# akashsengupta1997/STRAPS-3DHumanShapePose

Measured on AMD Instinct MI355X. Metric: bodies/sec, higher is better.
Workload: dtype fp32 (encoder convolutions as exact bf16x3 operand splits (six bf16 products per term); in-step SMPL blend contraction and skinning as 3-product fp16 splits (fp16x3_lbs: 22-bit operands); fp32 accumulate throughout)

## Files before the change

straps-3dhumanshapepose_amd/csrc/smpl_bwd.hip:

```cpp
#include "common.h"
#include "rodrigues.h"

namespace {

constexpr int KP = STRAPS_SMPL_KP, KG = KP / 8, NT = STRAPS_SMPL_TILES, NV = STRAPS_SMPL_V, NROUNDS = NT / 4;
constexpr int BT = 32, AS = 292, SS = 193;
constexpr int NJS = STRAPS_SMPL_NPICK + STRAPS_SMPL_NEXTRA;

__global__ __launch_bounds__(256, 1) STRAPS_NO_PACKED_FP32 void smpl_verts_bwd_kernel(straps_smpl_model_t m, const float* __restrict__ F,
                                                                const float* __restrict__ Amat, const float* __restrict__ dverts,
                                                                const float* __restrict__ djoints, float* __restrict__ dFp,
                                                                float* __restrict__ dAp, long long B, int rounds_per_chunk) {
    extern __shared__ __attribute__((aligned(16))) float smem[];
    float* As_ = smem;
    float* stage = As_ + BT * AS;

    const int tid = threadIdx.x, lane = tid & 63, wave = tid >> 6;
    const int h = lane >> 5, bl = lane & 31;
    const int chunk = blockIdx.x;
    const long long b0 = (long long)blockIdx.y * BT;
    const int nb = (int)((B - b0) < BT ? (B - b0) : BT);

    for (int i = tid; i < BT * 72; i += 256) {
        const int b = i / 72, q = i % 72;
        f32x4 v = {0.f, 0.f, 0.f, 0.f};
        if (b < nb) v = *reinterpret_cast<const f32x4*>(Amat + (b0 + b) * 288 + q * 4);
        *reinterpret_cast<f32x4*>(As_ + b * AS + q * 4) = v;
    }
    __syncthreads();

    const int round0 = chunk * rounds_per_chunk;
    const int round1 = min(round0 + rounds_per_chunk, NROUNDS);
    const f32x4* __restrict__ blend = reinterpret_cast<const f32x4*>(m.blend_frag);
    const f32x4* __restrict__ blend_t = reinterpret_cast<const f32x4*>(m.blend_frag_t);
    float* mystage = stage + wave * BT * SS;
    const int KW = m.skin_k;
    const bool vbody = bl < nb;

    float dacc[3][12];
#pragma unroll
    for (int i = 0; i < 3; ++i)
#pragma unroll
        for (int e = 0; e < 12; ++e) dacc[i][e] = 0.f;
    f32x16 accF[7];
#pragma unroll
    for (int f = 0; f < 7; ++f)
#pragma unroll
        for (int q = 0; q < 16; ++q) accF[f][q] = 0.f;

    for (int rd = round0; rd < round1; ++rd) {
        const int tile = rd * 4 + wave;
        f32x16 ax, ay, az;
#pragma unroll
        for (int r = 0; r < 16; ++r) { ax[r] = 0.f; ay[r] = 0.f; az[r] = 0.f; }
        {
            const f32x4* px = blend + ((long long)(tile * 3 + 0) * KG) * 64 + lane;
            const f32x4* py = px + KG * 64;
            const f32x4* pz = py + KG * 64;
            const float* frow = F + (b0 + (vbody ? bl : 0)) * KP + 4 * h;
            f32x4 cx0 = px[0], cy0 = py[0], cz0 = pz[0];
            f32x4 fn = *reinterpret_cast<const f32x4*>(frow);
#pragma unroll 2
            for (int g = 0; g < KG; ++g) {
                f32x4 nx0 = cx0, ny0 = cy0, nz0 = cz0;
                const f32x4 f0 = vbody ? fn : f32x4{0.f, 0.f, 0.f, 0.f};
                if (g + 1 < KG) {
                    nx0 = px[(g + 1) * 64]; ny0 = py[(g + 1) * 64]; nz0 = pz[(g + 1) * 64];
                    fn = *reinterpret_cast<const f32x4*>(frow + 8 * (g + 1));
                }
#pragma unroll
                for (int e = 0; e < 4; ++e) {
                    ax = mfma32(cx0[e], f0[e], ax);
                    ay = mfma32(cy0[e], f0[e], ay);
                    az = mfma32(cz0[e], f0[e], az);
                }
                cx0 = nx0; cy0 = ny0; cz0 = nz0;
            }
        }
        {
            const int ncol = min(96, (NV - tile * 32) * 3);
            for (int i = lane; i < BT * 96; i += 64) {
                const int b = i / 96, c = i - b * 96;
                float v = 0.f;
                if (dverts && b < nb && c < ncol) v = dverts[(b0 + b) * (long long)(NV * 3) + tile * 96 + c];
                mystage[b * SS + (c / 3) * 6 + (c % 3)] = v;
            }
        }
        __syncthreads();
        if (djoints && h == 0 && vbody) {
            const float* dj = djoints + (b0 + bl) * (STRAPS_SMPL_NJOINTS_OUT * 3) + 72;
            const int e0 = m.jrt_ptr[tile], e1 = m.jrt_ptr[tile + 1];
            for (int e = e0; e < e1; ++e) {
                const int code = m.jrt_code[e];
                const float w = m.jrt_w[e];
                float* sv = mystage + bl * SS + (code >> 8) * 6;
                const float* g = dj + (code & 255) * 3;
                sv[0] = fmaf(w, g[0], sv[0]); sv[1] = fmaf(w, g[1], sv[1]); sv[2] = fmaf(w, g[2], sv[2]);
            }
        }
        __syncthreads();
        {
            const float* Ab = As_ + bl * AS;
#pragma unroll
            for (int r = 0; r < 16; ++r) {
                const int vrow = (r & 3) + 8 * (r >> 2) + 4 * h;
                const int v = tile * 32 + vrow;
                float* sv = mystage + bl * SS + vrow * 6;
                const float gx = sv[0], gy = sv[1], gz = sv[2];
                sv[3] = ax[r]; sv[4] = ay[r]; sv[5] = az[r];
                float t00 = 0.f, t01 = 0.f, t02 = 0.f, t10 = 0.f, t11 = 0.f, t12 = 0.f, t20 = 0.f, t21 = 0.f, t22 = 0.f;
                for (int k = 0; k < KW; ++k) {
                    const float w = m.skin_w[v * KW + k];
                    const int jo = m.skin_j[v * KW + k] * 12;
                    const f32x4 a0 = *reinterpret_cast<const f32x4*>(Ab + jo);
                    const f32x4 a1 = *reinterpret_cast<const f32x4*>(Ab + jo + 4);
                    const f32x4 a2 = *reinterpret_cast<const f32x4*>(Ab + jo + 8);
                    t00 += w * a0[0]; t01 += w * a0[1]; t02 += w * a0[2];
                    t10 += w * a1[0]; t11 += w * a1[1]; t12 += w * a1[2];
                    t20 += w * a2[0]; t21 += w * a2[1]; t22 += w * a2[2];
                }
                ax[r] = t00 * gx + t10 * gy + t20 * gz;
                ay[r] = t01 * gx + t11 * gy + t21 * gz;
                az[r] = t02 * gx + t12 * gy + t22 * gz;
            }
        }
        __syncthreads();
#pragma unroll
        for (int i = 0; i < 3; ++i) {
            const int j = wave + 4 * (2 * i + h);
            const int e0 = m.dj_ptr[rd * 24 + j], e1 = m.dj_ptr[rd * 24 + j + 1];
            for (int e = e0; e < e1; ++e) {
                const int code = m.dj_code[e];
                const float w = m.dj_w[e];
                const float* sv = stage + ((code >> 5) * BT + bl) * SS + (code & 31) * 6;
                const float wx = w * sv[0], wy = w * sv[1], wz = w * sv[2];
                const float x = sv[3], y = sv[4], z = sv[5];
                dacc[i][0] = fmaf(wx, x, dacc[i][0]); dacc[i][1] = fmaf(wx, y, dacc[i][1]); dacc[i][2] = fmaf(wx, z, dacc[i][2]); dacc[i][3] += wx;
                dacc[i][4] = fmaf(wy, x, dacc[i][4]); dacc[i][5] = fmaf(wy, y, dacc[i][5]); dacc[i][6] = fmaf(wy, z, dacc[i][6]); dacc[i][7] += wy;
                dacc[i][8] = fmaf(wz, x, dacc[i][8]); dacc[i][9] = fmaf(wz, y, dacc[i][9]); dacc[i][10] = fmaf(wz, z, dacc[i][10]); dacc[i][11] += wz;
            }
        }
        {
            const f32x4* pt = blend_t + ((long long)tile * 3 * 7 * 4) * 64 + lane;
#pragma unroll
            for (int c = 0; c < 3; ++c) {
#pragma unroll
                for (int f = 0; f < 7; ++f) {
#pragma unroll
                    for (int rq = 0; rq < 4; ++rq) {
                        const f32x4 a = pt[((c * 7 + f) * 4 + rq) * 64];
#pragma unroll
                        for (int e = 0; e < 4; ++e) {
                            const float g = c == 0 ? ax[rq * 4 + e] : (c == 1 ? ay[rq * 4 + e] : az[rq * 4 + e]);
                            accF[f] = mfma32(a[e], g, accF[f]);
                        }
                    }
                }
            }
        }
        __syncthreads();
    }
    {
        __syncthreads();
        float* red = smem;
        if (wave >= 2) {
#pragma unroll
            for (int f = 0; f < 7; ++f)
#pragma unroll
                for (int q = 0; q < 16; ++q) red[(wave - 2) * 7168 + (f * 16 + q) * 64 + lane] = accF[f][q];
        }
        __syncthreads();
        if (wave < 2) {
#pragma unroll
            for (int f = 0; f < 7; ++f)
#pragma unroll
                for (int q = 0; q < 16; ++q) accF[f][q] += red[wave * 7168 + (f * 16 + q) * 64 + lane];
        }
        __syncthreads();
        if (wave == 1) {
#pragma unroll
            for (int f = 0; f < 7; ++f)
#pragma unroll
                for (int q = 0; q < 16; ++q) red[(f * 16 + q) * 64 + lane] = accF[f][q];
        }
        __syncthreads();
        if (wave == 0) {
#pragma unroll
            for (int f = 0; f < 7; ++f)
#pragma unroll
                for (int q = 0; q < 16; ++q) accF[f][q] += red[(f * 16 + q) * 64 + lane];
        }
    }
    if (vbody && wave == 0) {
        float* o = dFp + ((long long)chunk * B + b0 + bl) * KP;
#pragma unroll
        for (int f = 0; f < 7; ++f)
#pragma unroll
            for (int q = 0; q < 16; ++q) o[f * 32 + mfma_row(q, lane)] = accF[f][q];
    }
    if (vbody) {
        float* o = dAp + ((long long)chunk * B + b0 + bl) * 288;
#pragma unroll
        for (int i = 0; i < 3; ++i) {
            const int j = wave + 4 * (2 * i + h);
#pragma unroll
            for (int e = 0; e < 12; ++e) o[j * 12 + e] = dacc[i][e];
        }
    }
}

__device__ __forceinline__ float lane_get(float value, int src) { return __shfl(value, src, 64); }
template <bool AA>
__global__ __launch_bounds__(256) STRAPS_NO_PACKED_FP32 void smpl_pose_bwd_kernel(straps_smpl_model_t m, const float* __restrict__ betas,
                                                            const float* __restrict__ rotmats, const float* __restrict__ dFp,
                                                            const float* __restrict__ dAp, const float* __restrict__ djoints,
                                                            float* __restrict__ dbetas, float* __restrict__ drot, long long B,
                                                            int chunks, const float* __restrict__ aa, float* __restrict__ daa) {
    const int lane = threadIdx.x & 63;
    const int j = lane & 31;
    const int base = lane & 32;
    const long long body = ((long long)blockIdx.x * 256 + threadIdx.x) >> 5;
    const bool vb = body < B;
    const bool vj = j < 24;
    const long long bb = vb ? body : 0;
    const int jj = vj ? j : 0;

    float beta[10];
#pragma unroll
    for (int l = 0; l < 10; ++l) beta[l] = betas[bb * 10 + l];
    float R[9];
#pragma unroll
    for (int e = 0; e < 9; ++e) R[e] = rotmats[(bb * 24 + jj) * 9 + e];
    float J[3];
#pragma unroll
    for (int c = 0; c < 3; ++c) {
        float s = m.j_template[jj * 3 + c];
#pragma unroll
        for (int l = 0; l < 10; ++l) s = fmaf(m.j_shapedirs[(jj * 3 + c) * 10 + l], beta[l], s);
        J[c] = s;
    }
    const int par = m.parents[jj];
    const int dep = vj ? m.depth[jj] : -1;
    const int src = base + (par < 0 ? 0 : par);
    float rel[3];
#pragma unroll
    for (int c = 0; c < 3; ++c) {
        const float jp = lane_get(J[c], src);
        rel[c] = (jj > 0) ? J[c] - jp : J[c];
    }
    float G[12], PR[9];
#pragma unroll
    for (int r = 0; r < 3; ++r) {
        G[r * 4 + 0] = R[r * 3 + 0]; G[r * 4 + 1] = R[r * 3 + 1]; G[r * 4 + 2] = R[r * 3 + 2]; G[r * 4 + 3] = rel[r];
    }
#pragma unroll
    for (int e = 0; e < 9; ++e) PR[e] = (e == 0 || e == 4 || e == 8) ? 1.f : 0.f;
    for (int d = 1; d <= m.max_depth; ++d) {
        float P[12];
#pragma unroll
        for (int e = 0; e < 12; ++e) P[e] = lane_get(G[e], src);
        if (dep == d) {
#pragma unroll
            for (int r = 0; r < 3; ++r) {
                const float p0 = P[r * 4 + 0], p1 = P[r * 4 + 1], p2 = P[r * 4 + 2];
                PR[r * 3 + 0] = p0; PR[r * 3 + 1] = p1; PR[r * 3 + 2] = p2;
                G[r * 4 + 0] = p0 * R[0] + p1 * R[3] + p2 * R[6];
                G[r * 4 + 1] = p0 * R[1] + p1 * R[4] + p2 * R[7];
                G[r * 4 + 2] = p0 * R[2] + p1 * R[5] + p2 * R[8];
                G[r * 4 + 3] = p0 * rel[0] + p1 * rel[1] + p2 * rel[2] + P[r * 4 + 3];
            }
        }
    }
    float gA[12];
#pragma unroll
    for (int e = 0; e < 12; ++e) gA[e] = 0.f;
    if (vb && vj)
        for (int c = 0; c < chunks; ++c) {
            const float* p = dAp + (((long long)c * B + body) * 24 + j) * 12;
#pragma unroll
            for (int e = 0; e < 12; ++e) gA[e] += p[e];
        }
    float gGR[9], gGt[3], gJ[3];
#pragma unroll
    for (int r = 0; r < 3; ++r) {
        const float gat = gA[r * 4 + 3];
        gGR[r * 3 + 0] = gA[r * 4 + 0] - gat * J[0];
        gGR[r * 3 + 1] = gA[r * 4 + 1] - gat * J[1];
        gGR[r * 3 + 2] = gA[r * 4 + 2] - gat * J[2];
        gGt[r] = gat + ((vb && vj && djoints) ? djoints[(body * STRAPS_SMPL_NJOINTS_OUT + j) * 3 + r] : 0.f);
    }
#pragma unroll
    for (int c = 0; c < 3; ++c) gJ[c] = -(G[0 * 4 + c] * gA[3] + G[1 * 4 + c] * gA[7] + G[2 * 4 + c] * gA[11]);

    int child[3];
#pragma unroll
    for (int c = 0; c < 3; ++c) child[c] = m.children[jj * 3 + c];
    float gR[9];
#pragma unroll
    for (int e = 0; e < 9; ++e) gR[e] = 0.f;
    for (int d = m.max_depth; d >= 1; --d) {
        float M[15];
        const bool mine = (dep == d);
        float grel[3];
#pragma unroll
        for (int c = 0; c < 3; ++c) grel[c] = PR[0 * 3 + c] * gGt[0] + PR[1 * 3 + c] * gGt[1] + PR[2 * 3 + c] * gGt[2];
#pragma unroll
        for (int r = 0; r < 3; ++r)
#pragma unroll
            for (int c = 0; c < 3; ++c)
                M[r * 3 + c] = mine ? (gGR[r * 3 + 0] * R[c * 3 + 0] + gGR[r * 3 + 1] * R[c * 3 + 1] + gGR[r * 3 + 2] * R[c * 3 + 2] + gGt[r] * rel[c]) : 0.f;
#pragma unroll
        for (int c = 0; c < 3; ++c) { M[9 + c] = mine ? gGt[c] : 0.f; M[12 + c] = mine ? -grel[c] : 0.f; }
        if (mine) {
#pragma unroll
            for (int r = 0; r < 3; ++r)
#pragma unroll
                for (int c = 0; c < 3; ++c)
                    gR[r * 3 + c] = PR[0 * 3 + r] * gGR[0 * 3 + c] + PR[1 * 3 + r] * gGR[1 * 3 + c] + PR[2 * 3 + r] * gGR[2 * 3 + c];
#pragma unroll
            for (int c = 0; c < 3; ++c) gJ[c] += grel[c];
        }
#pragma unroll
        for (int cc = 0; cc < 3; ++cc) {
            const int ch = child[cc];
            const int cs = base + (ch < 0 ? 0 : ch);
            float in[15];
#pragma unroll
            for (int e = 0; e < 15; ++e) in[e] = lane_get(M[e], cs);
            if (vj && ch >= 0) {
#pragma unroll
                for (int e = 0; e < 9; ++e) gGR[e] += in[e];
#pragma unroll
                for (int c = 0; c < 3; ++c) { gGt[c] += in[9 + c]; gJ[c] += in[12 + c]; }
            }
        }
    }
    if (j == 0) {
#pragma unroll
        for (int e = 0; e < 9; ++e) gR[e] = gGR[e];
#pragma unroll
        for (int c = 0; c < 3; ++c) gJ[c] += gGt[c];
    }
    float gbeta_direct = 0.f;
    if (vb && vj) {
        for (int c = 0; c < chunks; ++c) {
            const float* p = dFp + ((long long)c * B + body) * KP;
            if (j >= 1) {
#pragma unroll
                for (int e = 0; e < 9; ++e) gR[e] += p[11 + (j - 1) * 9 + e];
            }
            if (j < 10) gbeta_direct += p[1 + j];
        }
        if (!AA || drot) {
#pragma unroll
            for (int e = 0; e < 9; ++e) drot[(body * 24 + j) * 9 + e] = gR[e];
        }
        if constexpr (AA) {
            float ox, oy, oz;
            const float* r = aa + (body * 24 + j) * 3;
            straps_rodrigues_bwd_one(r[0], r[1], r[2], gR, ox, oy, oz);
            float* o = daa + (body * 24 + j) * 3;
            o[0] = ox; o[1] = oy; o[2] = oz;
        }
    }
#pragma unroll
    for (int l = 0; l < 10; ++l) {
        float s = vj ? (m.j_shapedirs[(jj * 3 + 0) * 10 + l] * gJ[0] + m.j_shapedirs[(jj * 3 + 1) * 10 + l] * gJ[1] +
                        m.j_shapedirs[(jj * 3 + 2) * 10 + l] * gJ[2]) : 0.f;
#pragma unroll
        for (int o = 16; o > 0; o >>= 1) s += __shfl_xor(s, o, 64);
        const float direct = lane_get(gbeta_direct, base + l);
        if (vb && j == l) dbetas[body * 10 + l] = s + direct;
    }
}

inline int resolve_rpc(long long batch, int chunks) {
    if (chunks <= 0) chunks = (batch >= 1024) ? 8 : 54;
    if (chunks > NROUNDS) chunks = NROUNDS;
    return (NROUNDS + chunks - 1) / chunks;
}

}

int straps_smpl_launch_pose(const straps_smpl_model_t* model, const float* betas, const float* rotmats, float* F, float* Amat,
                            float* joints, long long batch, hipStream_t st);

extern "C" size_t straps_smpl_bwd_workspace_bytes(long long batch, int chunks) {
    const int rpc = resolve_rpc(batch, chunks);
    const int nch = (NROUNDS + rpc - 1) / rpc;
    return (size_t)batch * (size_t)(KP + 288 + nch * (KP + 288)) * sizeof(float);
}

namespace {
template <bool AA>
int smpl_bwd_launch(const straps_smpl_model_t* model, const float* betas, const float* rotmats, const float* aa, const float* dverts,
                    const float* djoints, float* dbetas, float* drotmats, float* daa, void* workspace, long long batch, int chunks,
                    void* stream) {
    hipStream_t st = (hipStream_t)stream;
    const int rpc = resolve_rpc(batch, chunks);
    const int nch = (NROUNDS + rpc - 1) / rpc;
    float* F = (float*)workspace;
    float* Amat = F + batch * KP;
    float* dFp = Amat + batch * 288;
    float* dAp = dFp + (long long)nch * batch * KP;
    int rc = straps_smpl_launch_pose(model, betas, rotmats, F, Amat, nullptr, batch, st);
    if (rc != STRAPS_OK) return rc;
    const size_t lds = (size_t)(BT * AS + 4 * BT * SS) * sizeof(float);
    STRAPS_RAISE_LDS((smpl_verts_bwd_kernel), lds, "smpl_verts_bwd_kernel");
    const long long btiles = (batch + BT - 1) / BT;
    if (btiles > 65535) { straps_set_error("straps_smpl_bwd: batch %lld exceeds one launch; split it", batch); return STRAPS_EUNSUPPORTED; }
    hipLaunchKernelGGL(smpl_verts_bwd_kernel, dim3(nch, (unsigned)btiles), dim3(256), lds, st, *model, F, Amat, dverts, djoints, dFp, dAp, batch, rpc);
    STRAPS_CHECK_LAUNCH("smpl_verts_bwd_kernel");
    hipLaunchKernelGGL(smpl_pose_bwd_kernel<AA>, dim3((unsigned)((batch * 32 + 255) / 256)), dim3(256), 0, st, *model, betas, rotmats, dFp, dAp,
                       djoints, dbetas, drotmats, batch, nch, aa, daa);
    STRAPS_CHECK_LAUNCH("smpl_pose_bwd_kernel");
    return STRAPS_OK;
}
}

extern "C" int straps_smpl_bwd(const straps_smpl_model_t* model, const float* betas, const float* rotmats, const float* dverts,
                               const float* djoints, float* dbetas, float* drotmats, void* workspace, long long batch, int chunks,
                               void* stream) {
    STRAPS_REQUIRE(model && betas && rotmats && dbetas && drotmats && workspace, "straps_smpl_bwd: null pointer");
    STRAPS_REQUIRE(model->blend_frag_t && model->children && model->jrt_ptr && model->dj_ptr && model->dj_code && model->dj_w,
                   "straps_smpl_bwd: model lacks the backward tables");
    STRAPS_REQUIRE(batch > 0, "straps_smpl_bwd: batch must be positive");
    return smpl_bwd_launch<false>(model, betas, rotmats, nullptr, dverts, djoints, dbetas, drotmats, nullptr, workspace, batch, chunks, stream);
}

extern "C" int straps_smpl_bwd_aa(const straps_smpl_model_t* model, const float* betas, const float* rotmats, const float* full_pose_aa,
                                  const float* dverts, const float* djoints, float* dbetas, float* dfull_pose_aa, float* drotmats,
                                  void* workspace, long long batch, int chunks, void* stream) {
    STRAPS_REQUIRE(model && betas && rotmats && full_pose_aa && dbetas && dfull_pose_aa && workspace, "straps_smpl_bwd_aa: null pointer");
    STRAPS_REQUIRE(model->blend_frag_t && model->children && model->jrt_ptr && model->dj_ptr && model->dj_code && model->dj_w,
                   "straps_smpl_bwd_aa: model lacks the backward tables");
    STRAPS_REQUIRE(batch > 0, "straps_smpl_bwd_aa: batch must be positive");
    return smpl_bwd_launch<true>(model, betas, rotmats, full_pose_aa, dverts, djoints, dbetas, drotmats, dfull_pose_aa, workspace, batch, chunks,
                                 stream);
}
```

Measured before the change: 7889.

## Software-pipeline SMPL backward loads with register rings and prefetched partial reductions

Restructures the vertex backward kernel so the blend and F operands are prefetched into RD-deep register rings with fully unrolled MFMA loops. The dverts tile is loaded into registers early and stored while the MFMAs run, and skinning weights and indices are preloaded. The blend_t MFMA stage also uses a RT-deep ring, the dj edge loop is batched in groups of EB, and __syncthreads is swapped for LDS-only fence barriers. The pose kernel now double-buffers the chunked dAp/dFp partial-sum reads in batches of PU. These changes are meant to hide global memory latency, at the cost of much higher register pressure and possible spills.

New measurement: 7979 (median of 6 runs). 1.01x the previous value.

```diff
diff --git a/straps-3dhumanshapepose_amd/csrc/smpl_bwd.hip b/straps-3dhumanshapepose_amd/csrc/smpl_bwd.hip
--- a/straps-3dhumanshapepose_amd/csrc/smpl_bwd.hip
+++ b/straps-3dhumanshapepose_amd/csrc/smpl_bwd.hip
@@ -6,6 +6,15 @@
 constexpr int KP = STRAPS_SMPL_KP, KG = KP / 8, NT = STRAPS_SMPL_TILES, NV = STRAPS_SMPL_V, NROUNDS = NT / 4;
 constexpr int BT = 32, AS = 292, SS = 193;
 constexpr int NJS = STRAPS_SMPL_NPICK + STRAPS_SMPL_NEXTRA;
+constexpr int RD = 4, RT = 4 * RD, SKP = 4, EB = 8;
+constexpr int PU = 9;
+static_assert(RD >= 1 && RT <= 84, "the rings are filled before their loops");
+
+__device__ __forceinline__ STRAPS_NO_PACKED_FP32 void lds_barrier() {
+    __builtin_amdgcn_fence(__ATOMIC_RELEASE, "workgroup", "local");
+    __builtin_amdgcn_s_barrier();
+    __builtin_amdgcn_fence(__ATOMIC_ACQUIRE, "workgroup", "local");
+}
 
 __global__ __launch_bounds__(256, 1) STRAPS_NO_PACKED_FP32 void smpl_verts_bwd_kernel(straps_smpl_model_t m, const float* __restrict__ F,
                                                                 const float* __restrict__ Amat, const float* __restrict__ dverts,
@@ -50,47 +59,84 @@
 
     for (int rd = round0; rd < round1; ++rd) {
         const int tile = rd * 4 + wave;
+        const f32x4* px = blend + ((long long)(tile * 3 + 0) * KG) * 64 + lane;
+        const f32x4* py = px + KG * 64;
+        const f32x4* pz = py + KG * 64;
+        int fo = (vbody ? bl : 0) * KP + 4 * h;
+        asm volatile("" : "+v"(fo));
+        const float* frow = F + b0 * KP + fo;
+        f32x4 rx[RD], ry[RD], rz[RD], rf[RD];
+#pragma unroll
+        for (int s = 0; s < RD; ++s) {
+            if (s < KG) {
+                rx[s] = px[s * 64]; ry[s] = py[s * 64]; rz[s] = pz[s * 64];
+                rf[s] = *reinterpret_cast<const f32x4*>(frow + 8 * s);
+            }
+        }
+        const int ncol = min(96, (NV - tile * 32) * 3);
+        const float* dvp[3];
+        int dvn[3], dvq[3], dvs[3];
+#pragma unroll
+        for (int u = 0; u < 3; ++u) {
+            const int i0 = lane + 64 * u, bu = i0 >= 96, c = i0 - 96 * bu;
+            dvn[u] = (dverts && c < ncol) ? (nb - bu + 1) / 2 : 0;
+            dvp[u] = dvn[u] > 0 ? dverts + (b0 + bu) * (long long)(NV * 3) + tile * 96 + c : F;
+            dvq[u] = dvn[u] > 0 ? 2 * NV * 3 : 0;
+            dvs[u] = bu * SS + (c / 3) * 6 + (c % 3);
+        }
+        float dvr[48];
+#pragma unroll
+        for (int q = 0; q < 16; ++q) {
+#pragma unroll
+            for (int u = 0; u < 3; ++u) dvr[3 * q + u] = dvp[u][min(q, max(dvn[u] - 1, 0)) * dvq[u]];
+        }
+        const int jr0 = m.jrt_ptr[tile], jr1 = m.jrt_ptr[tile + 1];
+        int de0[3], de1[3];
+#pragma unroll
+        for (int i = 0; i < 3; ++i) {
+            const int j = wave + 4 * (2 * i + h);
+            de0[i] = m.dj_ptr[rd * 24 + j]; de1[i] = m.dj_ptr[rd * 24 + j + 1];
+        }
         f32x16 ax, ay, az;
 #pragma unroll
         for (int r = 0; r < 16; ++r) { ax[r] = 0.f; ay[r] = 0.f; az[r] = 0.f; }
-        {
-            const f32x4* px = blend + ((long long)(tile * 3 + 0) * KG) * 64 + lane;
-            const f32x4* py = px + KG * 64;
-            const f32x4* pz = py + KG * 64;
-            const float* frow = F + (b0 + (vbody ? bl : 0)) * KP + 4 * h;
-            f32x4 cx0 = px[0], cy0 = py[0], cz0 = pz[0];
-            f32x4 fn = *reinterpret_cast<const f32x4*>(frow);
-#pragma unroll 2
-            for (int g = 0; g < KG; ++g) {
-                f32x4 nx0 = cx0, ny0 = cy0, nz0 = cz0;
-                const f32x4 f0 = vbody ? fn : f32x4{0.f, 0.f, 0.f, 0.f};
-                if (g + 1 < KG) {
-                    nx0 = px[(g + 1) * 64]; ny0 = py[(g + 1) * 64]; nz0 = pz[(g + 1) * 64];
-                    fn = *reinterpret_cast<const f32x4*>(frow + 8 * (g + 1));
-                }
-#pragma unroll
-                for (int e = 0; e < 4; ++e) {
-                    ax = mfma32(cx0[e], f0[e], ax);
-                    ay = mfma32(cy0[e], f0[e], ay);
-                    az = mfma32(cz0[e], f0[e], az);
-                }
-                cx0 = nx0; cy0 = ny0; cz0 = nz0;
-            }
-        }
-        {
-            const int ncol = min(96, (NV - tile * 32) * 3);
-            for (int i = lane; i < BT * 96; i += 64) {
-                const int b = i / 96, c = i - b * 96;
-                float v = 0.f;
-                if (dverts && b < nb && c < ncol) v = dverts[(b0 + b) * (long long)(NV * 3) + tile * 96 + c];
-                mystage[b * SS + (c / 3) * 6 + (c % 3)] = v;
-            }
-        }
-        __syncthreads();
+        __builtin_amdgcn_sched_barrier(0);
+#pragma unroll
+        for (int g = 0; g < KG; ++g) {
+            const int s = g % RD;
+            const f32x4 f0 = vbody ? rf[s] : f32x4{0.f, 0.f, 0.f, 0.f};
+#pragma unroll
+            for (int e = 0; e < 4; ++e) {
+                ax = mfma32(rx[s][e], f0[e], ax);
+                ay = mfma32(ry[s][e], f0[e], ay);
+                az = mfma32(rz[s][e], f0[e], az);
+            }
+            if (g + RD < KG) {
+                rx[s] = px[(g + RD) * 64]; ry[s] = py[(g + RD) * 64]; rz[s] = pz[(g + RD) * 64];
+                rf[s] = *reinterpret_cast<const f32x4*>(frow + 8 * (g + RD));
+            }
+            if (g == (RD < KG ? RD : KG) - 1) {
+#pragma unroll
+                for (int t = 0; t < 48; ++t)
+                    mystage[(t / 3) * 2 * SS + dvs[t % 3]] = t / 3 < dvn[t % 3] ? dvr[t] : 0.f;
+            }
+            __builtin_amdgcn_sched_barrier(0);
+        }
+        float skw[16][SKP];
+        int skj[16][SKP];
+#pragma unroll
+        for (int k = 0; k < SKP; ++k) {
+#pragma unroll
+            for (int r = 0; r < 16; ++r) {
+                const int v = tile * 32 + (r & 3) + 8 * (r >> 2) + 4 * h;
+                const int at = k < KW ? v * KW + k : 0;
+                skw[r][k] = m.skin_w[at]; skj[r][k] = m.skin_j[at];
+            }
+        }
+        lds_barrier();
         if (djoints && h == 0 && vbody) {
             const float* dj = djoints + (b0 + bl) * (STRAPS_SMPL_NJOINTS_OUT * 3) + 72;
-            const int e0 = m.jrt_ptr[tile], e1 = m.jrt_ptr[tile + 1];
-            for (int e = e0; e < e1; ++e) {
+            for (int e = jr0; e < jr1; ++e) {
                 const int code = m.jrt_code[e];
                 const float w = m.jrt_w[e];
                 float* sv = mystage + bl * SS + (code >> 8) * 6;
@@ -98,7 +144,7 @@
                 sv[0] = fmaf(w, g[0], sv[0]); sv[1] = fmaf(w, g[1], sv[1]); sv[2] = fmaf(w, g[2], sv[2]);
             }
         }
-        __syncthreads();
+        lds_barrier();
         {
             const float* Ab = As_ + bl * AS;
 #pragma unroll
@@ -109,7 +155,20 @@
                 const float gx = sv[0], gy = sv[1], gz = sv[2];
                 sv[3] = ax[r]; sv[4] = ay[r]; sv[5] = az[r];
                 float t00 = 0.f, t01 = 0.f, t02 = 0.f, t10 = 0.f, t11 = 0.f, t12 = 0.f, t20 = 0.f, t21 = 0.f, t22 = 0.f;
-                for (int k = 0; k < KW; ++k) {
+#pragma unroll
+                for (int k = 0; k < SKP; ++k) {
+                    if (k < KW) {
+                        const float w = skw[r][k];
+                        const int jo = skj[r][k] * 12;
+                        const f32x4 a0 = *reinterpret_cast<const f32x4*>(Ab + jo);
+                        const f32x4 a1 = *reinterpret_cast<const f32x4*>(Ab + jo + 4);
+                        const f32x4 a2 = *reinterpret_cast<const f32x4*>(Ab + jo + 8);
+                        t00 += w * a0[0]; t01 += w * a0[1]; t02 += w * a0[2];
+                        t10 += w * a1[0]; t11 += w * a1[1]; t12 += w * a1[2];
+                        t20 += w * a2[0]; t21 += w * a2[1]; t22 += w * a2[2];
+                    }
+                }
+                for (int k = SKP; k < KW; ++k) {
                     const float w = m.skin_w[v * KW + k];
                     const int jo = m.skin_j[v * KW + k] * 12;
                     const f32x4 a0 = *reinterpret_cast<const f32x4*>(Ab + jo);
@@ -119,46 +178,53 @@
                     t10 += w * a1[0]; t11 += w * a1[1]; t12 += w * a1[2];
                     t20 += w * a2[0]; t21 += w * a2[1]; t22 += w * a2[2];
                 }
-                ax[r] = t00 * gx + t10 * gy + t20 * gz;
-                ay[r] = t01 * gx + t11 * gy + t21 * gz;
-                az[r] = t02 * gx + t12 * gy + t22 * gz;
-            }
-        }
-        __syncthreads();
+                ax[r] = fmaf(t20, gz, fmaf(t00, gx, t10 * gy));
+                ay[r] = fmaf(t21, gz, fmaf(t01, gx, t11 * gy));
+                az[r] = fmaf(t22, gz, fmaf(t02, gx, t12 * gy));
+            }
+        }
+        const f32x4* pt = blend_t + ((long long)tile * 3 * 7 * 4) * 64 + lane;
+        f32x4 rt[RT];
+#pragma unroll
+        for (int s = 0; s < RT; ++s) rt[s] = pt[s * 64];
+        __builtin_amdgcn_sched_barrier(0);
+        lds_barrier();
 #pragma unroll
         for (int i = 0; i < 3; ++i) {
-            const int j = wave + 4 * (2 * i + h);
-            const int e0 = m.dj_ptr[rd * 24 + j], e1 = m.dj_ptr[rd * 24 + j + 1];
-            for (int e = e0; e < e1; ++e) {
-                const int code = m.dj_code[e];
-                const float w = m.dj_w[e];
-                const float* sv = stage + ((code >> 5) * BT + bl) * SS + (code & 31) * 6;
-                const float wx = w * sv[0], wy = w * sv[1], wz = w * sv[2];
-                const float x = sv[3], y = sv[4], z = sv[5];
-                dacc[i][0] = fmaf(wx, x, dacc[i][0]); dacc[i][1] = fmaf(wx, y, dacc[i][1]); dacc[i][2] = fmaf(wx, z, dacc[i][2]); dacc[i][3] += wx;
-                dacc[i][4] = fmaf(wy, x, dacc[i][4]); dacc[i][5] = fmaf(wy, y, dacc[i][5]); dacc[i][6] = fmaf(wy, z, dacc[i][6]); dacc[i][7] += wy;
-                dacc[i][8] = fmaf(wz, x, dacc[i][8]); dacc[i][9] = fmaf(wz, y, dacc[i][9]); dacc[i][10] = fmaf(wz, z, dacc[i][10]); dacc[i][11] += wz;
-            }
-        }
-        {
-            const f32x4* pt = blend_t + ((long long)tile * 3 * 7 * 4) * 64 + lane;
-#pragma unroll
-            for (int c = 0; c < 3; ++c) {
-#pragma unroll
-                for (int f = 0; f < 7; ++f) {
-#pragma unroll
-                    for (int rq = 0; rq < 4; ++rq) {
-                        const f32x4 a = pt[((c * 7 + f) * 4 + rq) * 64];
-#pragma unroll
-                        for (int e = 0; e < 4; ++e) {
-                            const float g = c == 0 ? ax[rq * 4 + e] : (c == 1 ? ay[rq * 4 + e] : az[rq * 4 + e]);
-                            accF[f] = mfma32(a[e], g, accF[f]);
-                        }
+            for (int e = de0[i]; e < de1[i]; e += EB) {
+                int code[EB];
+                float w[EB];
+#pragma unroll
+                for (int u = 0; u < EB; ++u) {
+                    const int at = min(e + u, de1[i] - 1);
+                    code[u] = m.dj_code[at]; w[u] = m.dj_w[at];
+                }
+#pragma unroll
+                for (int u = 0; u < EB; ++u) {
+                    if (e + u < de1[i]) {
+                        const float* sv = stage + ((code[u] >> 5) * BT + bl) * SS + (code[u] & 31) * 6;
+                        const float wx = w[u] * sv[0], wy = w[u] * sv[1], wz = w[u] * sv[2];
+                        const float x = sv[3], y = sv[4], z = sv[5];
+                        dacc[i][0] = fmaf(wx, x, dacc[i][0]); dacc[i][1] = fmaf(wx, y, dacc[i][1]); dacc[i][2] = fmaf(wx, z, dacc[i][2]); dacc[i][3] += wx;
+                        dacc[i][4] = fmaf(wy, x, dacc[i][4]); dacc[i][5] = fmaf(wy, y, dacc[i][5]); dacc[i][6] = fmaf(wy, z, dacc[i][6]); dacc[i][7] += wy;
+                        dacc[i][8] = fmaf(wz, x, dacc[i][8]); dacc[i][9] = fmaf(wz, y, dacc[i][9]); dacc[i][10] = fmaf(wz, z, dacc[i][10]); dacc[i][11] += wz;
                     }
                 }
             }
         }
-        __syncthreads();
+        __builtin_amdgcn_sched_barrier(0);
+#pragma unroll
+        for (int n = 0; n < 84; ++n) {
+            const int c = n / 28, f = (n / 4) % 7, rq = n % 4;
+#pragma unroll
+            for (int e = 0; e < 4; ++e) {
+                const float g = c == 0 ? ax[rq * 4 + e] : (c == 1 ? ay[rq * 4 + e] : az[rq * 4 + e]);
+                accF[f] = mfma32(rt[n % RT][e], g, accF[f]);
+            }
+            if (n + RT < 84) rt[n % RT] = pt[(n + RT) * 64];
+            __builtin_amdgcn_sched_barrier(0);
+        }
+        lds_barrier();
     }
     {
         __syncthreads();
@@ -210,6 +276,36 @@
 }
 
 __device__ __forceinline__ float lane_get(float value, int src) { return __shfl(value, src, 64); }
+__device__ __forceinline__ STRAPS_NO_PACKED_FP32 void pose_load_dA(float (&t)[PU][12], const float* p, long long stride) {
+#pragma unroll
+    for (int u = 0; u < PU; ++u)
+#pragma unroll
+        for (int e = 0; e < 12; ++e) t[u][e] = p[u * stride + e];
+}
+__device__ __forceinline__ STRAPS_NO_PACKED_FP32 void pose_add_dA(float (&gA)[12], const float (&t)[PU][12]) {
+#pragma unroll
+    for (int u = 0; u < PU; ++u)
+#pragma unroll
+        for (int e = 0; e < 12; ++e) gA[e] += t[u][e];
+}
+__device__ __forceinline__ STRAPS_NO_PACKED_FP32 void pose_load_dF(float (&t)[PU][10], const float* p, long long stride, int fR, int fB) {
+#pragma unroll
+    for (int u = 0; u < PU; ++u) {
+#pragma unroll
+        for (int e = 0; e < 9; ++e) t[u][e] = p[u * stride + fR + e];
+        t[u][9] = p[u * stride + fB];
+    }
+}
+__device__ __forceinline__ STRAPS_NO_PACKED_FP32 void pose_add_dF(float (&gR)[9], float& gbeta, const float (&t)[PU][10], bool rot, bool shape) {
+#pragma unroll
+    for (int u = 0; u < PU; ++u) {
+        if (rot) {
+#pragma unroll
+            for (int e = 0; e < 9; ++e) gR[e] += t[u][e];
+        }
+        if (shape) gbeta += t[u][9];
+    }
+}
 template <bool AA>
 __global__ __launch_bounds__(256) STRAPS_NO_PACKED_FP32 void smpl_pose_bwd_kernel(straps_smpl_model_t m, const float* __restrict__ betas,
                                                             const float* __restrict__ rotmats, const float* __restrict__ dFp,
@@ -224,6 +320,7 @@
     const bool vj = j < 24;
     const long long bb = vb ? body : 0;
     const int jj = vj ? j : 0;
+    const bool act = vb && vj;
 
     float beta[10];
 #pragma unroll
@@ -248,6 +345,11 @@
         const float jp = lane_get(J[c], src);
         rel[c] = (jj > 0) ? J[c] - jp : J[c];
     }
+    const float* pA = dAp + (bb * 24 + jj) * 12;
+    const long long sA = B * 288;
+    const int nbat = chunks / PU;
+    float tA[PU][12], tB[PU][12];
+    if (nbat > 0) pose_load_dA(tA, pA, sA);
     float G[12], PR[9];
 #pragma unroll
     for (int r = 0; r < 3; ++r) {
@@ -274,9 +376,17 @@
     float gA[12];
 #pragma unroll
     for (int e = 0; e < 12; ++e) gA[e] = 0.f;
-    if (vb && vj)
-        for (int c = 0; c < chunks; ++c) {
-            const float* p = dAp + (((long long)c * B + body) * 24 + j) * 12;
+#pragma unroll
+    for (int b = 0; b < NROUNDS / PU; ++b) {
+        if (b < nbat) {
+            const int bn = b + 1 < nbat ? b + 1 : b;
+            pose_load_dA(b & 1 ? tA : tB, pA + bn * PU * sA, sA);
+            pose_add_dA(gA, b & 1 ? tB : tA);
+        }
+    }
+    if (act)
+        for (int c = nbat * PU; c < chunks; ++c) {
+            const float* p = pA + c * sA;
 #pragma unroll
             for (int e = 0; e < 12; ++e) gA[e] += p[e];
         }
@@ -295,6 +405,11 @@
     int child[3];
 #pragma unroll
     for (int c = 0; c < 3; ++c) child[c] = m.children[jj * 3 + c];
+    const float* pF = dFp + bb * KP;
+    const long long sF = B * KP;
+    const int fR = 11 + (j >= 1 && vj ? j - 1 : 0) * 9, fB = 1 + (j < 10 ? j : 0);
+    float tF[PU][10], tG[PU][10];
+    if (nbat > 0) pose_load_dF(tF, pF, sF, fR, fB);
     float gR[9];
 #pragma unroll
     for (int e = 0; e < 9; ++e) gR[e] = 0.f;
@@ -342,8 +457,16 @@
         for (int c = 0; c < 3; ++c) gJ[c] += gGt[c];
     }
     float gbeta_direct = 0.f;
+#pragma unroll
+    for (int b = 0; b < NROUNDS / PU; ++b) {
+        if (b < nbat) {
+            const int bn = b + 1 < nbat ? b + 1 : b;
+            pose_load_dF(b & 1 ? tF : tG, pF + bn * PU * sF, sF, fR, fB);
+            pose_add_dF(gR, gbeta_direct, b & 1 ? tG : tF, j >= 1, j < 10);
+        }
+    }
     if (vb && vj) {
-        for (int c = 0; c < chunks; ++c) {
+        for (int c = nbat * PU; c < chunks; ++c) {
             const float* p = dFp + ((long long)c * B + body) * KP;
             if (j >= 1) {
 #pragma unroll
```
